# PIC4SeR/nav2_social_mpc_controller

Hardware: NVIDIA B200
Metric: mpc_solves_per_sec (higher is better)
Workload: dtype f64

## Files before the change

nav2_social_mpc_controller_b200/csrc/smpc_device.cuh:

```cuda
#pragma once
#include <cuda_runtime.h>
#include <stdint.h>

#include <cfloat>
#include <cmath>
#include <type_traits>

#include "smpc_math.cuh"

namespace smpc {

constexpr unsigned kFullMask = 0xffffffffu;
constexpr int kMaxSteps = 64;

struct DevParams {
  double w_distance, w_social, w_velocity, w_angle, w_agent_angle, w_prox, w_vf, w_obstacle, w_goal;
  double param_tol, fn_tol, gradient_tol;
  int max_iterations, ceres_compat, max_evaluations;
  int ch, bl, nb, n_bounded;
  int dof;
  int control_horizon, block_length;
};

struct DevBatch {
  int B, S, A, M, size_x, size_y;
  double resolution, dt;
  const double* pose0;
  const double* u0;
  const double* path_xy;
  const double* goal_yaw;
  const double* agents;
  const double* agents_packed;
  const uint8_t* agents_valid;
  const uint8_t* has_people;
  const uint8_t* costmaps;
  const double* costmap_origin;
  const int32_t* costmap_index;
  const int32_t* n_steps_each;
  unsigned* arrival;
  double* park_state;
  int* park_ring;
  int* park_counters;
  int park_quantum;
  int cta_sync;
  const int32_t* scenario;
  int n_rows;
};

struct DevResult {
  double* u;
  double* cmds;
  double* path;
  double* cost_initial;
  double* cost_final;
  int32_t* iterations;
  int32_t* termination;
  uint8_t* usable;
  int32_t* n_evals;
  double* trace;
  int trace_rows;
};

struct DevEvalOut {
  double* cost;
  double* cost_plain;
  double* grad;
  double* hess;
  uint8_t* ok;
};

struct Prob {
  double x0, y0, yaw0, goal_yaw, fin_x, fin_y, org_x, org_y;
  const double* px;
  const double* py;
  const double* agents;
  const double* packed;
  const uint8_t* valid;
  const uint8_t* map;
  int S, ch, bl, nb, nbd;
  bool has_people;
};

enum EvalFlags : unsigned { kResidualBad = 1u, kJacobianBad = 2u, kNoHessian = 4u };

__device__ __forceinline__ void add_masked(double& v, double t, double m) { v = fma(t, m, v); }

__device__ __forceinline__ double std_max(double a, double b) { return (a < b) ? b : a; }
__device__ __forceinline__ double std_min(double a, double b) { return (b < a) ? b : a; }

__device__ __forceinline__ double warp_sum(double v) {
#pragma unroll
  for (int d = 16; d > 0; d >>= 1) v += __shfl_xor_sync(kFullMask, v, d);
  return v;
}

struct PairOut {
  double fx, fy;
  double dfx[4], dfy[4];
  bool degenerate;
};

__device__ __forceinline__ double wrap_to_pi(double a) {
  while (a > M_PI) a -= 2.0 * M_PI;
  while (a <= -M_PI) a += 2.0 * M_PI;
  return a;
}

static __constant__ double kPairTab[6] = {0.35, 1.0 / 0.35, 2.1, 1e-6, 1e-12, 1e-9};

template <bool kReferenceAngle>
__device__ __forceinline__ void social_pair(double dx, double dy, double wx, double wy, PairOut& o) {
  const double kLambda = 2.0, kNPrime = 3.0, kN = 2.0;
  const double kGamma = kPairTab[0], kInvGamma = kPairTab[1], kFactor = kPairTab[2];
  double d2 = dx * dx + dy * dy;
  const bool tiny = d2 < kPairTab[4];
  if (kReferenceAngle && tiny) {
    dx = kPairTab[3];
    dy = 0.0;
    d2 = dx * dx;
  }
  const double inv_rho = rsqrt_pos(d2);
  const double rho = d2 * inv_rho;
  const double ex = dx * inv_rho, ey = dy * inv_rho;
  const double Ix = kLambda * wx + ex, Iy = kLambda * wy + ey;
  const double L2 = Ix * Ix + Iy * Iy;
  const double inv_L = rsqrt_pos(L2);
  const double L = L2 * inv_L;
  const double ix = Ix * inv_L, iy = Iy * inv_L;
  const double cross = ey * ix - ex * iy, dot = ex * ix + ey * iy;
  double theta;
  o.degenerate = tiny || !(fabs(cross) > kPairTab[5]);
  if (!kReferenceAngle || !o.degenerate) {
    theta = atan2_unit(cross, dot);
  } else {
    theta = wrap_to_pi(atan2(ey, ex) - atan2(iy, ix));
  }
  const double Bq = kGamma * L;
  const double inv_B = inv_L * kInvGamma;
  const double Bth = Bq * theta;
  const double t1 = kNPrime * Bth, t2 = kN * Bth;
  const double base = -rho * inv_B;
  const double E1 = exp_nonpos(base - t1 * t1);
  const double E2 = exp_nonpos(base - t2 * t2);
  const double fv = -E1, fa = kReferenceAngle ? ((theta > 0.0) ? -E2 : E2) : copysign(E2, -theta);
  const double Fix = kFactor * ix, Fiy = kFactor * iy;
  const double a = Fix * fv, b = Fiy * fa, c = Fiy * fv, d = Fix * fa;
  o.fx = a - b;
  o.fy = c + d;

  const double zd = (kReferenceAngle && tiny) ? 0.0 : 1.0;
  const double gr0 = zd * ex, gr1 = zd * ey;
  const double ge0 = -zd * ey * inv_rho, ge1 = zd * ex * inv_rho;
  const double k1 = -2.0 * t1 * kNPrime, k2 = -2.0 * t2 * kN;
  const double m1 = fma(a, k1, -(b * k2)), m2 = fma(c, k1, d * k2);
  const double thg = theta * kGamma;
  const double rho_BL = -base * inv_L;
  const double Xr = -inv_B * o.fx, Yr = -inv_B * o.fy;
  const double XL = fma(thg, m1, rho_BL * o.fx), YL = fma(thg, m2, rho_BL * o.fy);
  const double Xe = Bq * m1, Ye = Bq * m2;
  const double Xi = -Xe - o.fy, Yi = o.fx - Ye;
  const double cil = dot * inv_L;
  const double Xd = fma(Xi, cil, fma(XL, -cross, Xe)), Yd = fma(Yi, cil, fma(YL, -cross, Ye));
  o.dfx[0] = fma(Xd, ge0, Xr * gr0);
  o.dfx[1] = fma(Xd, ge1, Xr * gr1);
  o.dfy[0] = fma(Yd, ge0, Yr * gr0);
  o.dfy[1] = fma(Yd, ge1, Yr * gr1);
  const double lil = kLambda * inv_L;
  const double XLl = kLambda * XL, Xil = lil * Xi, YLl = kLambda * YL, Yil = lil * Yi;
  o.dfx[2] = fma(XLl, ix, -(Xil * iy));
  o.dfx[3] = fma(XLl, iy, Xil * ix);
  o.dfy[2] = fma(YLl, ix, -(Yil * iy));
  o.dfy[3] = fma(YLl, iy, Yil * ix);
}

static __device__ __noinline__ void social_pair_reference(double dx, double dy, double wx, double wy, double sign,
                                                          double* out) {
  PairOut o;
  social_pair<true>(dx, dy, wx, wy, o);
  out[0] = o.fx;
  out[1] = o.fy;
#pragma unroll
  for (int c = 0; c < 4; ++c) {
    out[2 + c] = sign * o.dfx[c];
    out[6 + c] = sign * o.dfy[c];
  }
}

__device__ __forceinline__ void hermite(double p0, double p1, double p2, double p3, double x, double& f, double& dfdx) {
  const double a = 0.5 * (-p0 + 3.0 * p1 - 3.0 * p2 + p3);
  const double b = 0.5 * (2.0 * p0 - 5.0 * p1 + 4.0 * p2 - p3);
  const double c = 0.5 * (-p0 + p2);
  f = p1 + x * (c + x * (b + x * a));
  dfdx = c + x * (2.0 * b + 3.0 * a * x);
}

template <bool NC, class T>
__device__ __forceinline__ T ld_in(const T* p) {
  if (NC) return __ldg(p);
  return __ldca(p);
}

template <bool NC>
__device__ __forceinline__ void bicubic(const uint8_t* map, int size_x, int size_y, double r, double c, double& f,
                                        double& dfdr, double& dfdc) {
  const double rf = floor(std_min(std_max(r, -4.0), (double)size_y + 4.0));
  const double cf = floor(std_min(std_max(c, -4.0), (double)size_x + 4.0));
  const int row = (int)rf, col = (int)cf;
  const double xr = r - (double)row, xc = c - (double)col;
  int cc[4];
#pragma unroll
  for (int k = 0; k < 4; ++k) cc[k] = min(max(col - 1 + k, 0), size_x - 1);
  double fr[4], dfr[4];
#pragma unroll
  for (int k = 0; k < 4; ++k) {
    const int rr = min(max(row - 1 + k, 0), size_y - 1);
    const uint8_t* line = map + (size_t)rr * size_x;
    hermite((double)ld_in<NC>(line + cc[0]), (double)ld_in<NC>(line + cc[1]), (double)ld_in<NC>(line + cc[2]),
            (double)ld_in<NC>(line + cc[3]), xc, fr[k], dfr[k]);
  }
  double unused;
  hermite(fr[0], fr[1], fr[2], fr[3], xr, f, dfdr);
  hermite(dfr[0], dfr[1], dfr[2], dfr[3], xr, dfdc, unused);
}

__device__ __forceinline__ int steps_in_block_before(int j, int beta, int bl, int last) {
  const int n = j - beta * bl;
  if (beta > last) return 0;
  if (beta == last) return max(n, 0);
  return min(max(n, 0), bl);
}

__device__ __forceinline__ double agent_angle_target(const DevBatch& bt, const Prob& pb, int step_plus_1) {
  const int stride = bt.S + 1;
  int closest = -1;
  double best = INFINITY;
  for (int k = 0; k < bt.A; ++k) {
    const double* a = pb.agents + (size_t)k * 6 * stride + step_plus_1;
    const double dx = a[0] - pb.x0, dy = a[stride] - pb.y0;
    const double d2 = dx * dx + dy * dy;
    if (d2 < best && a[4 * stride] > 0.05) {
      best = d2;
      closest = k;
    }
  }
  if (closest < 0 || best > 4.0) return NAN;
  const double* a = pb.agents + (size_t)closest * 6 * stride + step_plus_1;
  const double bearing = atan2(a[stride] - pb.y0, a[0] - pb.x0);
  const double hd_arg = a[2 * stride] - pb.yaw0;
  const double hd = atan2(sin(hd_arg), cos(hd_arg));
  const double wb_arg = bearing - pb.yaw0;
  const double wb = atan2(sin(wb_arg), cos(wb_arg));
  if (hd <= -(5 * M_PI / 6.0) || hd >= (M_PI / 6.0)) {
    if (wb < 0.0) return NAN;
    return pb.yaw0 + (-(M_PI / 6.0));
  }
  if (wb > 0.0) return NAN;
  return pb.yaw0 + (M_PI / 6.0);
}
#define SMPC_UNROLL _Pragma("unroll")
template <int G, class F>
__device__ __forceinline__ void scan_levels(F level) {
  if (G <= 8) {
    SMPC_UNROLL for (int d = 1; d < G; d <<= 1) level(d);
  } else {
    _Pragma("unroll 1") for (int d = 1; d < G; d <<= 1) level(d);
  }
}


constexpr int kRedStride = 33;

template <int NB, int D = 2>
struct Layout {
  static constexpr int P = D * NB;
  static constexpr int NH = P * (P + 1) / 2;
  static constexpr int NG = 2 + P;
  static constexpr int NE = NG + NH;
  static constexpr int NC = 4 + 4 * NB;
  static constexpr int kBuf0 = 0;
  static constexpr int kBuf1 = NE;
  static constexpr int kX = 2 * NE;
  static constexpr int kBest = kX + P;
  static constexpr int kScale = kBest + P;
  static constexpr int kDiag = kScale + P;
  static constexpr int kDelta = kDiag + P;
  static constexpr int kCand = kDelta + P;
  static constexpr int kCarry = kCand + P;
  static constexpr int kYaw = kCarry + NC;
  static constexpr int kState = kYaw + 2;
  static constexpr int kProb = kState + 22;
  static constexpr int kAa = kProb + 18;
  __host__ __device__ static constexpr int total(int S) { return ((kAa + S) | 1); }
  static constexpr int kRedDoubles = NE * kRedStride;
  __host__ __device__ static constexpr int g(int c) { return 2 + c; }
  __host__ __device__ static constexpr int h(int a, int b) { return NG + a * (a + 1) / 2 + b; }
};

__host__ __device__ constexpr int layout_total(int nb, int S, int dof = 2) {
  const int P = dof * nb, NE = 2 + P + P * (P + 1) / 2, NC = 4 + 4 * nb;
  return ((2 * NE + 6 * P + NC + 2 + 22 + 18 + S) | 1);
}
static_assert(layout_total(3, 28) == Layout<3>::total(28) && layout_total(5, 38) == Layout<5>::total(38) &&
                  layout_total(18, 18) == Layout<18>::total(18) && layout_total(3, 28, 3) == Layout<3, 3>::total(28),
              "layout_total must mirror Layout<NB>::total");

template <int G>
struct Group {
  static constexpr int kLog2 = (G == 32) ? 5 : (G == 16) ? 4 : (G == 8) ? 3 : (G == 4) ? 2 : (G == 2) ? 1 : 0;
  static constexpr int kPerWarp = 32 / G;
  __device__ static __forceinline__ unsigned mask(int lane) {
    return (G == 32) ? kFullMask : (((1u << G) - 1u) << (lane & ~(G - 1)));
  }
};

__device__ __forceinline__ double wrap_angle(double a) {
  return a - (2.0 * M_PI) * rint(a * (0.5 / M_PI));
}

enum Phase { kFetch = 0, kInit = 1, kLineSearch = 2, kFullStep = 3 };
struct LmState {
  double x_cost, x_norm, gmax, radius, decrease_factor, minimum_cost, it_cost, cost_initial, cost_final,
      model_cost_change, g0, dmax, t, prev_x, prev_value, prev_gradient;
  double se_cost;
  int iteration, n_invalid, n_eval, n_light, ls_iters, term, phase, b, flags, pad_;
};
static_assert(sizeof(LmState) == 22 * sizeof(double), "Layout::kState reserves 22 doubles");
static_assert(sizeof(Prob) <= 18 * sizeof(double), "Layout::kProb reserves 18 doubles");
enum StateFlags {
  kReuseDiagonal = 1, kItSuccessful = 2, kAnySuccess = 4, kPrevOk = 8, kLive = 16, kExhausted = 32, kSwapped = 64,
  kDrained = 128,
  kClosed = 256,
  kFinished = 512
};

template <int NB, int G, bool PPL, int D = 2>
__device__ __forceinline__ unsigned evaluate(const DevParams& prm, const DevBatch& bt, const Prob& pb, bool live,
                                             double* ws, double* red, const double* xs, int lane, double* out,
                                             const LmState* st) {
  using L = Layout<NB, D>;
  constexpr int P = L::P;
  const int gl = lane & (G - 1);
  const unsigned gmask = Group<G>::mask(lane);
  const int Sb = live ? pb.S : 0;
  const int Sw = (G == 32) ? Sb : __reduce_max_sync(kFullMask, Sb);
  const int bl = pb.bl, last_b = pb.nb - 1, ch = pb.ch;
  const double dt = bt.dt;
  const int stride = bt.S + 1;
  const double inv_res = 1.0 / bt.resolution;
  double* carry = ws + L::kCarry;
  const double* aa = ws + L::kAa;
  const int col0 = lane & ~(G - 1);
  unsigned flags = 0;
  bool need_h = true;
  bool bad_res = false, bad_jac = false;

  const double s0 = ws[L::kYaw], c0 = ws[L::kYaw + 1];

#pragma unroll 1
  for (int base = 0; base < Sw; base += G) {
    const int j = base + gl;
    const bool act = j < Sb;
    const bool first = (base == 0);
    const bool last = (base + G >= Sw);
    int bj = 0;
    SMPC_UNROLL for (int b = 1; b < NB; ++b) bj += (j >= b * bl && b <= last_b) ? 1 : 0;
    double vj = xs[0], wj = xs[D - 1];
    double vyj = 0.0;
    double Th = pb.yaw0;
    double tau[NB];
    SMPC_UNROLL for (int b = 0; b < NB; ++b) {
      if (b == bj) {
        vj = xs[D * b];
        wj = xs[D * b + D - 1];
        if (D == 3) vyj = xs[D * b + 1];
      }
      tau[b] = dt * (double)steps_in_block_before(j, b, bl, last_b);
      Th += xs[D * b + D - 1] * tau[b];
    }
    Th += wj * dt;
    double sT, cT;
    sincos(Th, &sT, &cT);
    double sn = __shfl_up_sync(kFullMask, sT, 1, G);
    double cs = __shfl_up_sync(kFullMask, cT, 1, G);
    if (gl == 0) {
      sn = first ? s0 : carry[2];
      cs = first ? c0 : carry[3];
    }
    const double cdt = act ? cs * dt : 0.0, sdt = act ? sn * dt : 0.0;
    const double aj = (D == 3) ? vj * cdt - vyj * sdt : vj * cdt;
    const double bjv = (D == 3) ? vj * sdt + vyj * cdt : vj * sdt;

    double sx = aj, sy = bjv;
    scan_levels<G>([&](int d) {
      const double tx = __shfl_up_sync(kFullMask, sx, d, G);
      const double ty = __shfl_up_sync(kFullMask, sy, d, G);
      const double m = (gl >= d) ? 1.0 : 0.0;
      add_masked(sx, tx, m);
      add_masked(sy, ty, m);
    });
    const double X = (first ? pb.x0 : carry[0]) + sx;
    const double Y = (first ? pb.y0 : carry[1]) + sy;

    double ra = 0.0, caT = 0.0;
    double rs = 0.0, sX = 0.0, sY = 0.0, sTh = 0.0, sL = 0.0;
    double sM = 0.0;
    double rp = 0.0, pX = 0.0, pY = 0.0;
    double cprox_plain = 0.0;
    if (PPL && act && pb.has_people) {
      const double tgt = aa[j];
      if (tgt == tgt) {
        const double del = wrap_angle(Th - tgt);
        ra = prm.w_agent_angle * (del * del);
        caT = 2.0 * prm.w_agent_angle * del;
      }
      const double rvx = (D == 3) ? vj * cT - vyj * sT : vj * cT;
      const double rvy = (D == 3) ? vj * sT + vyj * cT : vj * sT;
      double Frx = 0.0, Fry = 0.0;
      double JFx[4] = {0, 0, 0, 0}, JFy[4] = {0, 0, 0, 0};
      double wp = 0.0;
      double G4[4] = {0, 0, 0, 0};
      double dmin = DBL_MAX, pdx = 0.0, pdy = 0.0;
      const bool do_social = prm.w_social != 0.0;
      const double2* rec = reinterpret_cast<const double2*>(pb.packed) + ((size_t)(j + 1)) * 2;
      const uint8_t* vld = pb.valid + (j + 1);
      double2 nxt_p = __ldg(rec);
      double2 nxt_v = __ldg(rec + 1);
      unsigned char nxt_valid = __ldg(vld);
#ifndef SMPC_PAIR_UNROLL
#define SMPC_PAIR_UNROLL 1
#endif
      constexpr int kPairUnroll = SMPC_PAIR_UNROLL;
#pragma unroll kPairUnroll
      for (int k = 0; k < bt.A; ++k) {
        const double ax = nxt_p.x, ay = nxt_p.y, avx = nxt_v.x, avy = nxt_v.y;
        const bool valid = nxt_valid != 0;
        if (k + 1 < bt.A) {
          rec += (size_t)stride * 2;
          vld += stride;
          nxt_p = __ldg(rec);
          nxt_v = __ldg(rec + 1);
          nxt_valid = __ldg(vld);
        }
        const double ddx = X - ax, ddy = Y - ay;
        {
          const double d2 = ddx * ddx + ddy * ddy;
          const bool closer = valid && d2 < dmin;
          dmin = closer ? d2 : dmin;
          pdx = closer ? ddx : pdx;
          pdy = closer ? ddy : pdy;
        }
        if (do_social) {
          PairOut po;
          social_pair<false>(ddx, ddy, rvx - avx, rvy - avy, po);
          const bool degenerate = po.degenerate;
          if (degenerate) {
            double ref[10];
            social_pair_reference(ddx, ddy, rvx - avx, rvy - avy, 1.0, ref);
            po.fx = ref[0];
            po.fy = ref[1];
            SMPC_UNROLL for (int c = 0; c < 4; ++c) {
              po.dfx[c] = ref[2 + c];
              po.dfy[c] = ref[6 + c];
            }
          }
          {
            const double m = valid ? 1.0 : 0.0;
            Frx = fma(m, po.fx, Frx);
            Fry = fma(m, po.fy, Fry);
            SMPC_UNROLL for (int c = 0; c < 4; ++c) {
              JFx[c] = fma(m, po.dfx[c], JFx[c]);
              JFy[c] = fma(m, po.dfy[c], JFy[c]);
            }
          }
          if (degenerate) {
            double ref[10];
            social_pair_reference(-ddx, -ddy, avx - rvx, avy - rvy, -1.0, ref);
            po.fx = ref[0];
            po.fy = ref[1];
            SMPC_UNROLL for (int c = 0; c < 4; ++c) {
              po.dfx[c] = ref[2 + c];
              po.dfy[c] = ref[6 + c];
            }
          }
          wp = fma(po.fy, po.fy, fma(po.fx, po.fx, wp));
          SMPC_UNROLL for (int c = 0; c < 4; ++c) G4[c] = fma(po.fy, po.dfy[c], fma(po.fx, po.dfx[c], G4[c]));
        }
      }
      if (do_social) {
        const double wr = Frx * Frx + Fry * Fry;
        SMPC_UNROLL for (int c = 0; c < 4; ++c) G4[c] = 2.0 * fma(Fry, JFy[c], fma(Frx, JFx[c], G4[c]));
        rs = prm.w_social * (wr + wp + 1e-6);
        sX = prm.w_social * G4[0];
        sY = prm.w_social * G4[1];
        sL = prm.w_social * (G4[2] * cT + G4[3] * sT);
        if (D == 3) {
          sM = prm.w_social * (-G4[2] * sT + G4[3] * cT);
          sTh = prm.w_social * (-G4[2] * rvy + G4[3] * rvx);
        } else {
          sTh = prm.w_social * vj * (-G4[2] * sT + G4[3] * cT);
        }
      }
      const double r_true = (dmin == DBL_MAX) ? 0.0 : prm.w_prox * (3.0 * exp(-dmin / (0.5 * 0.5)));
      cprox_plain = 0.5 * r_true * r_true;
      if (prm.ceres_compat < 210) {
        rp = prm.w_prox * 3.0;
      } else if (dmin == DBL_MAX) {
        flags |= kJacobianBad;
      } else {
        rp = r_true;
        const double k = -r_true * (2.0 / (0.5 * 0.5));
        pX = k * pdx;
        pY = k * pdy;
      }
    }

    double sd[4 * NB];
    SMPC_UNROLL for (int b = 0; b < NB; ++b) {
      sd[4 * b + 0] = (b == bj) ? cdt : 0.0;
      sd[4 * b + 1] = (b == bj) ? sdt : 0.0;
      sd[4 * b + 2] = -bjv * tau[b];
      sd[4 * b + 3] = aj * tau[b];
    }
    scan_levels<G>([&](int d) {
      const double m = (gl >= d) ? 1.0 : 0.0;
      SMPC_UNROLL for (int e = 0; e < 4 * NB; ++e) add_masked(sd[e], __shfl_up_sync(kFullMask, sd[e], d, G), m);
    });
    if (!first) {
      SMPC_UNROLL for (int e = 0; e < 4 * NB; ++e) sd[e] += carry[4 + e];
    }
    if (!last) {
      __syncwarp(gmask);
      if (gl == G - 1) {
        carry[0] = X;
        carry[1] = Y;
        carry[2] = sT;
        carry[3] = cT;
        SMPC_UNROLL for (int e = 0; e < 4 * NB; ++e) carry[4 + e] = sd[e];
      }
      __syncwarp(gmask);
    }

    auto column = [&](int pa, double& cx, double& cy, double& c3) -> int {
      const int ba = pa / D, k = pa % D;
      if (k == D - 1) {
        cx = sd[4 * ba + 2];
        cy = sd[4 * ba + 3];
        c3 = tau[ba] + ((ba == bj) ? dt : 0.0);
        return 2;
      }
      c3 = (ba == bj) ? 1.0 : 0.0;
      if (k == 0) {
        cx = sd[4 * ba + 0];
        cy = sd[4 * ba + 1];
        return 0;
      }
      cx = -sd[4 * ba + 1];
      cy = sd[4 * ba + 0];
      return 1;
    };
    double mXX = 0, mXY = 0, mXT = 0, mXL = 0, mYY = 0, mYT = 0, mYL = 0, mTT = 0, mTL = 0, mLL = 0;
    double qX = 0, qY = 0, qT = 0, qL = 0;
    double mXM = 0, mYM = 0, mTM = 0, mLM = 0, mMM = 0, qM = 0;
    if (act) {
      double cost = 0.0;
      if (PPL) {
        cost += 0.5 * ra * ra;
        mTT += caT * caT;
        qT += caT * ra;
        cost += 0.5 * rs * rs;
        mXX += sX * sX; mXY += sX * sY; mXT += sX * sTh; mXL += sX * sL;
        mYY += sY * sY; mYT += sY * sTh; mYL += sY * sL;
        mTT += sTh * sTh; mTL += sTh * sL; mLL += sL * sL;
        qX += sX * rs; qY += sY * rs; qT += sTh * rs; qL += sL * rs;
        if (D == 3) {
          mXM += sX * sM; mYM += sY * sM; mTM += sTh * sM; mLM += sL * sM; mMM += sM * sM;
          qM += sM * rs;
        }
        mXX += pX * pX; mXY += pX * pY; mYY += pY * pY;
        qX += pX * rp; qY += pY * rp;
      }
      if (j < ch) {
        const double e = 0.6 - vj;
        if (D == 3) {
          const double r = prm.w_velocity * e * e + prm.w_velocity * vyj * vyj;
          const double cL = -2.0 * prm.w_velocity * e, cM = 2.0 * prm.w_velocity * vyj;
          cost += 0.5 * r * r;
          mLL += cL * cL; mLM += cL * cM; mMM += cM * cM;
          qL += cL * r; qM += cM * r;
        } else {
          const double r = prm.w_velocity * e * e;
          const double cL = -2.0 * prm.w_velocity * e;
          cost += 0.5 * r * r;
          mLL += cL * cL;
          qL += cL * r;
        }
      }
      {
        const double turn = wrap_angle(pb.goal_yaw - Th);
        const double r = prm.w_goal * turn * turn;
        const double cTh = -2.0 * prm.w_goal * turn;
        cost += 0.5 * r * r;
        mTT += cTh * cTh;
        qT += cTh * r;
      }
      {
        const double ex = X - pb.fin_x, ey = Y - pb.fin_y;
        const double q2 = ex * ex + ey * ey;
        const double r = prm.w_distance * q2 * q2;
        const double k = 4.0 * prm.w_distance * q2;
        const double cX = k * ex, cY = k * ey;
        cost += 0.5 * r * r;
        mXX += cX * cX; mXY += cX * cY; mYY += cY * cY;
        qX += cX * r; qY += cY * r;
      }
      {
        const double ex = X - ld_in<PPL>(pb.px + j + 1), ey = Y - ld_in<PPL>(pb.px + stride + j + 1);
        const double q2 = ex * ex + ey * ey;
        const double r = prm.w_angle * q2 * q2;
        const double k = 4.0 * prm.w_angle * q2;
        const double cX = k * ex, cY = k * ey;
        cost += 0.5 * r * r;
        mXX += cX * cX; mXY += cX * cY; mYY += cY * cY;
        qX += cX * r; qY += cY * r;
      }
      {
        const double fxw = X + 0.25 * cT, fyw = Y + 0.25 * sT;
        const double gx = (fxw - pb.org_x) * inv_res, gy = (fyw - pb.org_y) * inv_res;
        double f, dfdr, dfdc;
        bicubic<PPL>(pb.map, bt.size_x, bt.size_y, gy, gx, f, dfdr, dfdc);
        const double r = prm.w_obstacle * f;
        const double kx = prm.w_obstacle * dfdc * inv_res, ky = prm.w_obstacle * dfdr * inv_res;
        const double cTh = 0.25 * (-kx * sT + ky * cT);
        cost += 0.5 * r * r;
        mXX += kx * kx; mXY += kx * ky; mXT += kx * cTh;
        mYY += ky * ky; mYT += ky * cTh; mTT += cTh * cTh;
        qX += kx * r; qY += ky * r; qT += cTh * r;
      }

      {
        const double c_diff = cost + 0.5 * rp * rp, c_plain = cost + cprox_plain;
        double* r0 = red + lane;
        auto put_g = [&](auto is_first) {
          constexpr bool kFirst = decltype(is_first)::value;
          r0[0 * kRedStride] = (kFirst ? 0.0 : r0[0 * kRedStride]) + c_diff;
          r0[1 * kRedStride] = (kFirst ? 0.0 : r0[1 * kRedStride]) + c_plain;
          SMPC_UNROLL for (int pa = 0; pa < P; ++pa) {
            double cx, cy, cs3;
            const int kind = column(pa, cx, cy, cs3);
            double* gp = r0 + L::g(pa) * kRedStride;
            *gp = (kFirst ? 0.0 : *gp) + (qX * cx + qY * cy + ((kind == 0) ? qL : (kind == 1) ? qM : qT) * cs3);
          }
        };
        if (first) put_g(std::true_type{}); else put_g(std::false_type{});
      }
    } else if (first) {
      SMPC_UNROLL for (int e = 0; e < L::NG; ++e) red[e * kRedStride + lane] = 0.0;
    }

    if (last) {
      if (gl == 0 && live) {
        SMPC_UNROLL for (int i = 1; i < NB; ++i) {
          if (i < pb.nbd) {
            double dk[D], r = 0.0;
            SMPC_UNROLL for (int k = 0; k < D; ++k) {
              dk[k] = xs[D * i + k] - xs[D * (i - 1) + k];
              r += prm.w_vf * dk[k] * dk[k];
            }
            red[0 * kRedStride + lane] += 0.5 * r * r;
            red[1 * kRedStride + lane] += 0.5 * r * r;
            SMPC_UNROLL for (int k = 0; k < D; ++k) {
              const double jk = 2.0 * prm.w_vf * dk[k];
              red[L::g(D * (i - 1) + k) * kRedStride + lane] -= jk * r;
              red[L::g(D * i + k) * kRedStride + lane] += jk * r;
            }
          }
        }
      }
      __syncwarp();
      for (int e = gl; e < L::NG; e += G) {
        const double* row = red + e * kRedStride + col0;
        double t0 = 0.0, t1 = 0.0;
        SMPC_UNROLL for (int t = 0; t < G; t += 2) {
          t0 += row[t];
          t1 += row[t + 1];
        }
        const double tot = t0 + t1;
        out[e] = tot;
        if (!isfinite(tot)) {
          if (e < 2) bad_res = true; else bad_jac = true;
        }
      }
      if (__any_sync(gmask, bad_res)) flags |= kResidualBad;
      if (__any_sync(gmask, bad_jac)) flags |= kJacobianBad;
      flags = __reduce_or_sync(gmask, flags);
      __syncwarp(gmask);
      if (st != nullptr && live && st->phase == kLineSearch) {
        const bool armijo_ok = (flags == 0) && !(out[0] > st->x_cost + 1e-4 * st->g0 * st->t);
        need_h = armijo_ok;
      }
    }

    if (need_h) {
      if (act) {
        double* r0 = red + lane;
        auto put_h = [&](auto is_first) {
          constexpr bool kFirst = decltype(is_first)::value;
          SMPC_UNROLL for (int pa = 0; pa < P; ++pa) {
            double ax, ay, as3;
            const int ka = column(pa, ax, ay, as3);
            const double t0 = mXX * ax + mXY * ay + ((ka == 0) ? mXL : (ka == 1) ? mXM : mXT) * as3;
            const double t1 = mXY * ax + mYY * ay + ((ka == 0) ? mYL : (ka == 1) ? mYM : mYT) * as3;
            const double t2 = mXT * ax + mYT * ay + ((ka == 0) ? mTL : (ka == 1) ? mTM : mTT) * as3;
            const double t3 = mXL * ax + mYL * ay + ((ka == 0) ? mLL : (ka == 1) ? mLM : mTL) * as3;
            const double t4 = mXM * ax + mYM * ay + ((ka == 0) ? mLM : (ka == 1) ? mMM : mTM) * as3;
            SMPC_UNROLL for (int pb2 = 0; pb2 <= pa; ++pb2) {
              double bx, by, bs3;
              const int kb = column(pb2, bx, by, bs3);
              double* p = r0 + L::h(pa, pb2) * kRedStride;
              *p = (kFirst ? 0.0 : *p) + (bx * t0 + by * t1 + bs3 * ((kb == 0) ? t3 : (kb == 1) ? t4 : t2));
            }
          }
        };
        if (first) put_h(std::true_type{}); else put_h(std::false_type{});
      } else if (first) {
        SMPC_UNROLL for (int e = L::NG; e < L::NE; ++e) red[e * kRedStride + lane] = 0.0;
      }
    }
  }

  if (need_h) {
    if (gl == 0 && live) {
      SMPC_UNROLL for (int i = 1; i < NB; ++i) {
        if (i < pb.nbd) {
          double jk[D];
          SMPC_UNROLL for (int k = 0; k < D; ++k) jk[k] = 2.0 * prm.w_vf * (xs[D * i + k] - xs[D * (i - 1) + k]);
          SMPC_UNROLL for (int k = 0; k < D; ++k) {
            SMPC_UNROLL for (int l = 0; l < D; ++l) {
              const double v = jk[k] * jk[l];
              if (l <= k) {
                red[(L::h(D * i + k, D * i + l)) * kRedStride + lane] += v;
                red[(L::h(D * (i - 1) + k, D * (i - 1) + l)) * kRedStride + lane] += v;
              }
              red[(L::h(D * i + k, D * (i - 1) + l)) * kRedStride + lane] -= v;
            }
          }
        }
      }
    }
  }
  __syncwarp();
  if (need_h) {
    bool bad_h = false;
    for (int e = L::NG + gl; e < L::NE; e += G) {
      const double* row = red + e * kRedStride + col0;
      double t0 = 0.0, t1 = 0.0;
      SMPC_UNROLL for (int t = 0; t < G; t += 2) {
        t0 += row[t];
        t1 += row[t + 1];
      }
      const double tot = t0 + t1;
      out[e] = tot;
      if (!isfinite(tot)) bad_h = true;
    }
    if (__any_sync(gmask, bad_h)) flags |= kJacobianBad;
  } else {
    flags |= kNoHessian;
  }
  __syncwarp();
  return flags;
}

struct LsSample {
  double x, value, gradient;
  bool ok;
};

__device__ __forceinline__ double horner5(const double (&m)[6], double x) {
  return m[0] + x * (m[1] + x * (m[2] + x * (m[3] + x * (m[4] + x * m[5]))));
}

static __device__ __noinline__ void quartic_aberth(const double* c, double* re) {
  double m[5];
  for (int i = 0; i <= 4; ++i) m[i] = c[4 - i] / c[4];
  double radius = 0.0;
  for (int i = 1; i <= 4; ++i) radius = fmax(radius, pow(fabs(m[i]), 1.0 / i));
  radius = 2.0 * radius + 1e-300;
  double zr[4], zi[4];
  for (int i = 0; i < 4; ++i) {
    double s, co;
    sincos(2.0 * M_PI * i / 4 + 0.35, &s, &co);
    zr[i] = 0.7 * radius * co;
    zi[i] = 0.7 * radius * s;
  }
  for (int it = 0; it < 60; ++it) {
    double moved = 0.0;
    for (int i = 0; i < 4; ++i) {
      double pr = m[0], pi = 0.0, dr = 0.0, di = 0.0;
      for (int j = 1; j <= 4; ++j) {
        const double ndr = dr * zr[i] - di * zi[i] + pr, ndi = dr * zi[i] + di * zr[i] + pi;
        const double npr = pr * zr[i] - pi * zi[i] + m[j], npi = pr * zi[i] + pi * zr[i];
        dr = ndr; di = ndi; pr = npr; pi = npi;
      }
      if (pr == 0.0 && pi == 0.0) continue;
      const double dn = dr * dr + di * di;
      const double rr = (pr * dr + pi * di) / dn, ri = (pi * dr - pr * di) / dn;
      double sr = 0.0, si = 0.0;
      for (int j = 0; j < 4; ++j) {
        if (j == i) continue;
        const double er = zr[i] - zr[j], ei = zi[i] - zi[j];
        const double en = er * er + ei * ei;
        sr += er / en;
        si -= ei / en;
      }
      const double qr = 1.0 - (rr * sr - ri * si), qi = -(rr * si + ri * sr);
      const double qn = qr * qr + qi * qi;
// ... 796 lines not shown
```

Baseline: 877,800.

## Software-pipeline social pair loop by splitting front and back halves

Splits the social-force pair computation into a front stage (normalisation, angle) and a back stage (exponentials, derivatives), then interleaves the front of agent k+1 with the back of agent k. The goal is more instruction-level parallelism across the long dependent chain of rsqrt, atan2 and exp. It also tracks the nearest agent by index and reloads its position later instead of carrying dx/dy, and defers the agent-angle load and the initial yaw loads. In exchange it raises register pressure, which may lower occupancy, and adds reloads on the degenerate and proximity paths.

```diff
diff --git a/nav2_social_mpc_controller_b200/csrc/smpc_device.cuh b/nav2_social_mpc_controller_b200/csrc/smpc_device.cuh
--- a/nav2_social_mpc_controller_b200/csrc/smpc_device.cuh
+++ b/nav2_social_mpc_controller_b200/csrc/smpc_device.cuh
@@ -94,10 +94,17 @@
   return v;
 }
 
+struct PairFront {
+  double ex, ey, inv_rho, rho;
+  double ix, iy, inv_L, L;
+  double theta;
+  bool tiny;
+  bool degenerate;
+};
+
 struct PairOut {
   double fx, fy;
   double dfx[4], dfy[4];
-  bool degenerate;
 };
 
 __device__ __forceinline__ double wrap_to_pi(double a) {
@@ -109,9 +116,8 @@
 static __constant__ double kPairTab[6] = {0.35, 1.0 / 0.35, 2.1, 1e-6, 1e-12, 1e-9};
 
 template <bool kReferenceAngle>
-__device__ __forceinline__ void social_pair(double dx, double dy, double wx, double wy, PairOut& o) {
-  const double kLambda = 2.0, kNPrime = 3.0, kN = 2.0;
-  const double kGamma = kPairTab[0], kInvGamma = kPairTab[1], kFactor = kPairTab[2];
+__device__ __forceinline__ void pair_front(double dx, double dy, double wx, double wy, PairFront& p) {
+  const double kLambda = 2.0;
   double d2 = dx * dx + dy * dy;
   const bool tiny = d2 < kPairTab[4];
   if (kReferenceAngle && tiny) {
@@ -128,13 +134,32 @@
   const double L = L2 * inv_L;
   const double ix = Ix * inv_L, iy = Iy * inv_L;
   const double cross = ey * ix - ex * iy, dot = ex * ix + ey * iy;
-  double theta;
-  o.degenerate = tiny || !(fabs(cross) > kPairTab[5]);
-  if (!kReferenceAngle || !o.degenerate) {
-    theta = atan2_unit(cross, dot);
+  p.degenerate = tiny || !(fabs(cross) > kPairTab[5]);
+  if (!kReferenceAngle || !p.degenerate) {
+    p.theta = atan2_unit(cross, dot);
   } else {
-    theta = wrap_to_pi(atan2(ey, ex) - atan2(iy, ix));
-  }
+    p.theta = wrap_to_pi(atan2(ey, ex) - atan2(iy, ix));
+  }
+  p.ex = ex;
+  p.ey = ey;
+  p.inv_rho = inv_rho;
+  p.rho = rho;
+  p.ix = ix;
+  p.iy = iy;
+  p.inv_L = inv_L;
+  p.L = L;
+  p.tiny = tiny;
+}
+
+template <bool kReferenceAngle>
+__device__ __forceinline__ void pair_back(const PairFront& p, PairOut& o) {
+  const double kLambda = 2.0, kNPrime = 3.0, kN = 2.0;
+  const double kGamma = kPairTab[0], kInvGamma = kPairTab[1], kFactor = kPairTab[2];
+  const double ex = p.ex, ey = p.ey, inv_rho = p.inv_rho, rho = p.rho;
+  const double ix = p.ix, iy = p.iy, inv_L = p.inv_L, L = p.L;
+  const double theta = p.theta;
+  const bool tiny = p.tiny;
+  const double cross = ey * ix - ex * iy, dot = ex * ix + ey * iy;
   const double Bq = kGamma * L;
   const double inv_B = inv_L * kInvGamma;
   const double Bth = Bq * theta;
@@ -174,15 +199,17 @@
 }
 
 static __device__ __noinline__ void social_pair_reference(double dx, double dy, double wx, double wy, double sign,
-                                                          double* out) {
+                                                          PairOut& out) {
+  PairFront p;
+  pair_front<true>(dx, dy, wx, wy, p);
   PairOut o;
-  social_pair<true>(dx, dy, wx, wy, o);
-  out[0] = o.fx;
-  out[1] = o.fy;
+  pair_back<true>(p, o);
+  out.fx = o.fx;
+  out.fy = o.fy;
 #pragma unroll
   for (int c = 0; c < 4; ++c) {
-    out[2 + c] = sign * o.dfx[c];
-    out[6 + c] = sign * o.dfy[c];
+    out.dfx[c] = sign * o.dfx[c];
+    out.dfy[c] = sign * o.dfy[c];
   }
 }
 
@@ -354,7 +381,7 @@
   bool need_h = true;
   bool bad_res = false, bad_jac = false;
 
-  const double s0 = ws[L::kYaw], c0 = ws[L::kYaw + 1];
+  const double s0 = PPL ? 0.0 : ws[L::kYaw], c0 = PPL ? 0.0 : ws[L::kYaw + 1];
 
 #pragma unroll 1
   for (int base = 0; base < Sw; base += G) {
@@ -383,8 +410,8 @@
     double sn = __shfl_up_sync(kFullMask, sT, 1, G);
     double cs = __shfl_up_sync(kFullMask, cT, 1, G);
     if (gl == 0) {
-      sn = first ? s0 : carry[2];
-      cs = first ? c0 : carry[3];
+      sn = first ? (PPL ? ws[L::kYaw] : s0) : carry[2];
+      cs = first ? (PPL ? ws[L::kYaw + 1] : c0) : carry[3];
     }
     const double cdt = act ? cs * dt : 0.0, sdt = act ? sn * dt : 0.0;
     const double aj = (D == 3) ? vj * cdt - vyj * sdt : vj * cdt;
@@ -407,84 +434,88 @@
     double rp = 0.0, pX = 0.0, pY = 0.0;
     double cprox_plain = 0.0;
     if (PPL && act && pb.has_people) {
-      const double tgt = aa[j];
-      if (tgt == tgt) {
-        const double del = wrap_angle(Th - tgt);
-        ra = prm.w_agent_angle * (del * del);
-        caT = 2.0 * prm.w_agent_angle * del;
-      }
       const double rvx = (D == 3) ? vj * cT - vyj * sT : vj * cT;
       const double rvy = (D == 3) ? vj * sT + vyj * cT : vj * sT;
       double Frx = 0.0, Fry = 0.0;
       double JFx[4] = {0, 0, 0, 0}, JFy[4] = {0, 0, 0, 0};
       double wp = 0.0;
       double G4[4] = {0, 0, 0, 0};
-      double dmin = DBL_MAX, pdx = 0.0, pdy = 0.0;
+      double dmin = DBL_MAX;
+      int kmin = 0;
       const bool do_social = prm.w_social != 0.0;
-      const double2* rec = reinterpret_cast<const double2*>(pb.packed) + ((size_t)(j + 1)) * 2;
+      const int A = bt.A;
+      auto agent_record = [&](int k) { return reinterpret_cast<const double2*>(pb.packed) + ((size_t)k * stride + j + 1) * 2; };
+      const double2* rec = agent_record(0);
       const uint8_t* vld = pb.valid + (j + 1);
-      double2 nxt_p = __ldg(rec);
-      double2 nxt_v = __ldg(rec + 1);
-      unsigned char nxt_valid = __ldg(vld);
-#ifndef SMPC_PAIR_UNROLL
-#define SMPC_PAIR_UNROLL 1
-#endif
-      constexpr int kPairUnroll = SMPC_PAIR_UNROLL;
-#pragma unroll kPairUnroll
-      for (int k = 0; k < bt.A; ++k) {
-        const double ax = nxt_p.x, ay = nxt_p.y, avx = nxt_v.x, avy = nxt_v.y;
-        const bool valid = nxt_valid != 0;
-        if (k + 1 < bt.A) {
-          rec += (size_t)stride * 2;
-          vld += stride;
-          nxt_p = __ldg(rec);
-          nxt_v = __ldg(rec + 1);
-          nxt_valid = __ldg(vld);
-        }
-        const double ddx = X - ax, ddy = Y - ay;
+      auto next_agent = [&](int k, double& ddx, double& ddy, double& wx, double& wy) {
+        const double2 np = __ldg(rec), nv = __ldg(rec + 1);
+        const bool valid = __ldg(vld) != 0;
+        rec += (size_t)stride * 2;
+        vld += stride;
+        const double ax = np.x, ay = np.y, avx = nv.x, avy = nv.y;
+        ddx = X - ax;
+        ddy = Y - ay;
+        wx = rvx - avx;
+        wy = rvy - avy;
+        const double d2 = ddx * ddx + ddy * ddy;
+        const bool closer = valid && d2 < dmin;
+        dmin = closer ? d2 : dmin;
+        kmin = closer ? k : kmin;
+        return valid;
+      };
+      if (!do_social) {
+        for (int k = 0; k < A; ++k) {
+          double ddx, ddy, wx, wy;
+          next_agent(k, ddx, ddy, wx, wy);
+        }
+      } else if (A > 0) {
+        auto finish_agent = [&](int k, bool degenerate, bool valid, const PairOut& po) {
+          const double m = valid ? 1.0 : 0.0;
+          auto add = [&](const PairOut& on_robot, const PairOut& on_agent) {
+            Frx = fma(m, on_robot.fx, Frx);
+            Fry = fma(m, on_robot.fy, Fry);
+            SMPC_UNROLL for (int c = 0; c < 4; ++c) {
+              JFx[c] = fma(m, on_robot.dfx[c], JFx[c]);
+              JFy[c] = fma(m, on_robot.dfy[c], JFy[c]);
+            }
+            wp = fma(on_agent.fy, on_agent.fy, fma(on_agent.fx, on_agent.fx, wp));
+            SMPC_UNROLL for (int c = 0; c < 4; ++c)
+              G4[c] = fma(on_agent.fy, on_agent.dfy[c], fma(on_agent.fx, on_agent.dfx[c], G4[c]));
+          };
+          if (!degenerate) {
+            add(po, po);
+          } else {
+            const double2* r = agent_record(k);
+            const double2 p = __ldg(r), v = __ldg(r + 1);
+            const double ddx = X - p.x, ddy = Y - p.y;
+            PairOut on_robot, on_agent;
+            social_pair_reference(ddx, ddy, rvx - v.x, rvy - v.y, 1.0, on_robot);
+            social_pair_reference(-ddx, -ddy, v.x - rvx, v.y - rvy, -1.0, on_agent);
+            add(on_robot, on_agent);
+          }
+        };
+        PairFront cur;
+        bool cur_valid;
         {
-          const double d2 = ddx * ddx + ddy * ddy;
-          const bool closer = valid && d2 < dmin;
-          dmin = closer ? d2 : dmin;
-          pdx = closer ? ddx : pdx;
-          pdy = closer ? ddy : pdy;
-        }
-        if (do_social) {
+          double ddx, ddy, wx, wy;
+          cur_valid = next_agent(0, ddx, ddy, wx, wy);
+          pair_front<false>(ddx, ddy, wx, wy, cur);
+        }
+#pragma unroll 1
+        for (int k = 0; k + 1 < A; ++k) {
           PairOut po;
-          social_pair<false>(ddx, ddy, rvx - avx, rvy - avy, po);
-          const bool degenerate = po.degenerate;
-          if (degenerate) {
-            double ref[10];
-            social_pair_reference(ddx, ddy, rvx - avx, rvy - avy, 1.0, ref);
-            po.fx = ref[0];
-            po.fy = ref[1];
-            SMPC_UNROLL for (int c = 0; c < 4; ++c) {
-              po.dfx[c] = ref[2 + c];
-              po.dfy[c] = ref[6 + c];
-            }
-          }
-          {
-            const double m = valid ? 1.0 : 0.0;
-            Frx = fma(m, po.fx, Frx);
-            Fry = fma(m, po.fy, Fry);
-            SMPC_UNROLL for (int c = 0; c < 4; ++c) {
-              JFx[c] = fma(m, po.dfx[c], JFx[c]);
-              JFy[c] = fma(m, po.dfy[c], JFy[c]);
-            }
-          }
-          if (degenerate) {
-            double ref[10];
-            social_pair_reference(-ddx, -ddy, avx - rvx, avy - rvy, -1.0, ref);
-            po.fx = ref[0];
-            po.fy = ref[1];
-            SMPC_UNROLL for (int c = 0; c < 4; ++c) {
-              po.dfx[c] = ref[2 + c];
-              po.dfy[c] = ref[6 + c];
-            }
-          }
-          wp = fma(po.fy, po.fy, fma(po.fx, po.fx, wp));
-          SMPC_UNROLL for (int c = 0; c < 4; ++c) G4[c] = fma(po.fy, po.dfy[c], fma(po.fx, po.dfx[c], G4[c]));
-        }
+          pair_back<false>(cur, po);
+          double ddx, ddy, wx, wy;
+          const bool nxt_ok = next_agent(k + 1, ddx, ddy, wx, wy);
+          PairFront nxt;
+          pair_front<false>(ddx, ddy, wx, wy, nxt);
+          finish_agent(k, cur.degenerate, cur_valid, po);
+          cur = nxt;
+          cur_valid = nxt_ok;
+        }
+        PairOut po;
+        pair_back<false>(cur, po);
+        finish_agent(A - 1, cur.degenerate, cur_valid, po);
       }
       if (do_social) {
         const double wr = Frx * Frx + Fry * Fry;
@@ -509,8 +540,15 @@
       } else {
         rp = r_true;
         const double k = -r_true * (2.0 / (0.5 * 0.5));
-        pX = k * pdx;
-        pY = k * pdy;
+        const double2 p = __ldg(agent_record(kmin));
+        pX = k * (X - p.x);
+        pY = k * (Y - p.y);
+      }
+      const double tgt = aa[j];
+      if (tgt == tgt) {
+        const double del = wrap_angle(Th - tgt);
+        ra = prm.w_agent_angle * (del * del);
+        caT = 2.0 * prm.w_agent_angle * del;
       }
     }
 
```

New measurement: 818,800 (median of 6 runs). -6.7%, worse.
